# pierre-haessig/stodynprog

Measured on AMD Instinct MI355X. Metric: vi_sweeps_per_sec, higher is better.
Workload: dtype f64

## Files before the change

### stodynprog_amd/codegen.py

```python
import hashlib
import re
import math
import os

import numpy as np

from .trace import TracedModel, DEP_X

CSRC = os.path.join(os.path.dirname(os.path.abspath(__file__)), 'csrc')


DEBUG_INT_MACROS = ('SDP_COL_SHARE_X2', 'SDP_COL_MIN_WAVES', 'SDP_COL_BATCH', 'SDP_COL_WMODE', 'SDP_COL_UNROLL_U', 'SDP_COL_UNROLL_W',
                    'SDP_COL_A_GROUP', 'SDP_COL_A_ORDER', 'SDP_COL_FILTER_UNROLL', 'SDP_COL_B_PRIO',
                    'SDP_COL_FILTER_TOP2', 'SDP_COL_TILE', 'SDP_COL_FILTER_RUNROLL', 'SDP_COL_LEAN', 'SDP_COL_WIDE',
                    'SDP_COL_A_WIDE_LOADS', 'SDP_COLU_WIDE_LOADS', 'SDP_COLU_A_GROUP', 'SDP_COL_LDS_PAD', 'SDP_COL_HOIST',
                    'SDP_COL_TAIL_KEEP', 'SDP_COL_KEEP_BATCH', 'SDP_COL_KEEP_LOADS', 'SDP_COL_TAIL_HOLD', 'SDP_SHORT_GROUP', 'SDP_BNB_CHUNK')
DEBUG_NAMES = frozenset(DEBUG_INT_MACROS + (
    'SDP_STAMP', 'SDP_NO_POW2', 'SDP_EXTRA_DEFINES', 'SDP_COL_FILTER_SCALE', 'SDP_LEAD_FILTER_SCALE',
    'SDP_LEAD_UNROLL', 'SDP_COL_A_LW', 'SDP_COL_FILTER', 'SDP_COL_SHIFT', 'SDP_COL_UTAB', 'SDP_LEAD_FILTER',
    'SDP_COL_THREADS', 'SDP_COL_WCHUNK', 'SDP_STG_CU', 'SDP_COL_WPAIR', 'SDP_COL_WRES', 'SDP_COL_LEAN2', 'SDP_COL_BNB',
    'SDP_LINE_FILTER', 'SDP_LINE_FILTER_SCALE', 'SDP_LINE_TOP2'))


def check_debug(debug):
    if not debug:
        return None
    unknown = sorted(set(debug) - DEBUG_NAMES)
    if unknown:
        raise ValueError('unknown debug define(s): {}'.format(', '.join(unknown)))
    return {k: str(v) for k, v in debug.items() if v is not None and str(v) != ''} or None


def _dbg(debug, name, default=None):
    if not debug:
        return default
    v = debug.get(name)
    return default if v is None or str(v) == '' else str(v)

_BIN_INFIX = {'add': '+', 'sub': '-', 'mul': '*', 'div': '/',
              'lt': '<', 'le': '<=', 'gt': '>', 'ge': '>=', 'eq': '==', 'ne': '!=',
              'and': '&&', 'or': '||', 'xor': '!='}
_FUNC1 = {'abs': 'fabs', 'sqrt': 'sqrt', 'floor': 'floor', 'ceil': 'ceil', 'trunc': 'trunc',
          'rint': 'rint', 'exp': 'exp', 'exp2': 'exp2', 'expm1': 'expm1', 'log': 'log',
          'log2': 'log2', 'log10': 'log10', 'log1p': 'log1p', 'sin': 'sin', 'cos': 'cos',
          'tan': 'tan', 'asin': 'asin', 'acos': 'acos', 'atan': 'atan', 'sinh': 'sinh',
          'cosh': 'cosh', 'tanh': 'tanh', 'cbrt': 'cbrt'}
_FUNC2 = {'pow': 'pow', 'atan2': 'atan2', 'hypot': 'hypot', 'fmod': 'fmod',
          'min': 'sdp_npmin', 'max': 'sdp_npmax', 'fmin': 'sdp_npfmin', 'fmax': 'sdp_npfmax',
          'pymod': 'sdp_nppymod', 'floordiv': 'sdp_npfloordiv'}


def real_literal(value):
    if math.isnan(value):
        return '(sdp_real)NAN'
    if math.isinf(value):
        return '(sdp_real)INFINITY' if value > 0 else '(-(sdp_real)INFINITY)'
    return '(sdp_real)({})'.format(float(value).hex())


def _emit_node(n, name, param_index=None):
    a = [name(x) for x in n.args]
    op = n.op
    if op == 'const':
        if param_index is not None and n.id in param_index:
            return 'sdp_model_prm[{}]'.format(param_index[n.id])
        return real_literal(n.value)
    if op == 'bconst':
        return 'true' if n.value else 'false'
    if op == 'var':
# ... 322 lines not shown
    return lines


def _column_lines(model, dtype, column, col_cfg, window, per_control, filtered, utab, debug, wres=0):
    rs = np.dtype(dtype).itemsize
    wpair = use_wpair(model, dtype, debug) and window is None
    shifted = bool(filtered and column_shift_applies(model, dtype, debug=debug))
    lines = ['#define SDP_COST_HAS_W {}'.format(1 if model.cost_depends_on_w else 0),
             '#define SDP_LEAD_HAS_W {}'.format(1 if model.lead_depends_on_w else 0),
             '#define SDP_TRAIL_HAS_U {}'.format(1 if model.trail_depends_on_u else 0),
             '#define SDP_COL_N0 {}'.format(int(column[0])),
             '#define SDP_COL_W {}'.format(max(int(column[1]), 1)),
             '#define SDP_COL_THREADS {}'.format(col_cfg[0]),
             '#define SDP_COL_WPAIR {}'.format(1 if wpair else 0)]
    if wres:
        lines.append('#define SDP_COL_WRES {}         // resident-chunk form: perturbation points the table holds at a time'.format(int(wres)))
        if rs == 8 and shifted and not _dbg(debug, 'SDP_COL_UNROLL_W'):
            lines.append('#define SDP_COL_UNROLL_W 1')
    if filtered and int(col_cfg[0]) <= 256 and not _dbg(debug, 'SDP_COL_MIN_WAVES'):
        if wres:
            lines.append('#define SDP_COL_MIN_WAVES {}    // as many waves per SIMD as the LDS image admits workgroups per CU, at most 4'.format(
                max(1, min(4, (COLUMN_LDS_MAX // int(col_cfg[1])) * int(col_cfg[0]) // 256))))
        else:
            lines.append('#define SDP_COL_MIN_WAVES 1    // small workgroups of the filtered kernel: no register cap')
    if filtered:
        lines.append('#define SDP_COL_FILTER 1')
        if shifted:
            lines += ['#define SDP_COL_SHIFT 1        // x0\' = a(x, u) +- b_1(x_1.., w) +- ..: first pass on the shifted lattice',
                      '#define SDP_COL_SHIFT_TERMS {}'.format(len(model.lead_split()[1])),
                      '#define SDP_COL_SHIFT_CHAIN {}        // additions of a chain of sums that was regrouped (0: the final-sum form)'.format(
                          model.lead_split_chain()[1] if model.lead_split_chain() is not None else 0),
                      '#define SDP_COL_SHIFT_ROWS {}'.format(int(col_cfg[2]))]
        if _dbg(debug, 'SDP_COL_FILTER_SCALE'):
            lines.append('#define SDP_COL_FILTER_SCALE {}'.format(float(_dbg(debug, 'SDP_COL_FILTER_SCALE'))))
    if per_control is None and not _dbg(debug, 'SDP_COL_A_ORDER'):
        wide = column_wide_loads(column[0], dtype, window, debug)
        order = column_build_order(int(col_cfg[0]), column[1], int(window[2]) if window is not None else column[0],
                                   (16 // rs) if wide else 1)
        if order[0] == 2:
            lw = int(_dbg(debug, 'SDP_COL_A_LW') or order[1])
            lines += ['#define SDP_COL_A_ORDER 2',
                      '#define SDP_COL_A_LW {}'.format(lw)]
            if rs == 4 and int(column[0]) >= 512 and not wres and window is None and not _dbg(debug, 'SDP_COL_A_GROUP'):
                lines.append('#define SDP_COL_A_GROUP 8      // table entries per thread whose vertex loads are issued together')
            if wide and not _dbg(debug, 'SDP_COL_A_WIDE_LOADS'):
                lines.append('#define SDP_COL_A_WIDE_LOADS 1')

                if (wres and rs == 8 and not wpair and window is None and _dbg(debug, 'SDP_COL_TAIL_HOLD') is None
                        and not _dbg(debug, 'SDP_COL_TAIL_KEEP')):
                    tail, groups = int(column[1]) - int(wres), int(col_cfg[0]) // lw
                    if (tail > 0 and tail % groups == 0 and int(column[0]) % (2 * lw) == 0
                            and (tail // groups) * (int(column[0]) // (2 * lw)) * 4 <= 32):
                        lines.append('#define SDP_COL_TAIL_HOLD 1    // the tail of the table is built once and held in registers')
    if window is not None:
        lines.append('#define SDP_COL_ROWS {}'.format(int(window[2])))
    if per_control is not None:
        lines.append('#define SDP_COL_WCHUNK {}'.format(int(per_control[2])))
        if int(column[0]) % (16 // rs) == 0 and not _dbg(debug, 'SDP_COLU_WIDE_LOADS'):
            lines.append('#define SDP_COLU_WIDE_LOADS 1')
    for k in DEBUG_INT_MACROS:
        if _dbg(debug, k):
            lines.append('#define {} {}'.format(k, int(_dbg(debug, k))))
    lines += [separable_functions_source(model), '']
    if utab is not None and filtered:
        lines += ['#define SDP_COL_UTAB {}'.format(len(utab[0])),
                  '#define SDP_COL_UTAB_N {}'.format(int(utab[1])),
                  control_table_source(model, utab[0]), '']
        short = None
        if not model.cost_depends_on_w and window is None and per_control is None \
                and _dbg(debug, 'SDP_COL_LEAN2') != '0' and (not shifted or rs == 8):
            if rs == 8 and wres and _dbg(debug, 'SDP_COL_LEAN') != '0':
                short = short_pass_source(model, utab[0], 'SDP_COL_LEAN2')
                if short and _dbg(debug, 'SDP_COL_BNB') != '0':
                    short += ('\n#define SDP_COL_BNB 1          // the short first pass as a certified branch and bound over '
                              'blocks of controls (sdp_lean2_bnb)')

            elif rs == 4 and not wres and _dbg(debug, 'SDP_COL_WIDE') != '0' and _dbg(debug, 'SDP_COL_LEAN') in (None, '0') \
                    and _dbg(debug, 'SDP_COL_FILTER_TOP2') in (None, '1'):
                short = short_pass_source(model, utab[0], 'SDP_COL_WIDE2')
                if short and _dbg(debug, 'SDP_COL_BNB') != '0':
                    short += ('\n#define SDP_COL_BNB 1          // the short wide first pass as a certified branch and bound over '
                              'blocks of controls (sdp_short_bnb)')
                    if int(column[0]) >= 512 and not _dbg(debug, 'SDP_BNB_CHUNK'):
                        short += '\n#define SDP_BNB_CHUNK 4        // blocks whose bounds are evaluated together (see SDP_COL_A_GROUP above)'
        if short:
            lines += [short, '']
    lines += ['#include "sdp_column_kernel.h"    // also brings in sdp_sweep_kernel.h', '']
    return lines


def line_filter_applies(model, dtype, W, debug=None):
    if _dbg(debug, 'SDP_LINE_FILTER', '1') == '0':
        return False
    return bool(model.n_state == 1 and model.n_perturb == 1 and 1 <= int(W) <= 1024 and np.dtype(dtype).itemsize == 8
                and not model.time_dep and model.lead_depends_on_w and not model.cost_depends_on_w
                and model.lead_split() is not None)


def line_functions_source(model):
    a_node, terms = model.lead_split()
    out = []
    lines = ['SDP_DEV sdp_real sdp_model_lead_a(const sdp_real *x, const sdp_real *u, sdp_real t)',
             '{', '    (void)x; (void)u; (void)t;']
    names = _emit_body(model, model.slice_nodes([a_node]), lines)
    lines += ['    return {};'.format(names[a_node.id]), '}']
    out.append('\n'.join(lines))
# ... 264 lines not shown
    else:
        whole = _column_lds(w, w, n0, n_state, rs, threads, reduced=True, utab_values=utab_values)
        part = _column_lds(half, w, n0, n_state, rs, threads, reduced=True, utab_values=utab_values)
    if COLUMN_LDS_MAX // whole < 3 <= COLUMN_LDS_MAX // part:
        return half if RESIDENT_CHUNKS_DEFAULT else 0
    return 0


RESIDENT_CHUNKS_DEFAULT = True


def column_wide_loads(n0, dtype, window, debug=None):
    if _dbg(debug, 'SDP_COL_A_WIDE_LOADS', '1') == '0':
        return False
    rpl = 16 // np.dtype(dtype).itemsize
    if rpl != 2 and _dbg(debug, 'SDP_COL_A_WIDE_LOADS') != '1':
        return False
    return int(n0) % rpl == 0 and window is None


def column_build_order(threads, w, rows, rows_per_lane=1):
    w = max(int(w), 1)
    best = (0, 0, 0.0)
    for lw in ((32, 64, 16, 8) if rows_per_lane > 1 else (64, 32, 16, 8)):
        if lw * rows_per_lane > rows or threads % lw:
            continue
        groups = threads // lw
        util = w / float(-(-w // groups) * groups)
        if util > best[2] + 1e-9:
            best = (2, lw, util)
    return (best[0], best[1]) if best[2] >= 0.85 else (0, 0)


def bnb_words(n_controls):
    n = max(int(n_controls), 1)
    block = 8
    while (n + block - 1) // block > 64:
        block *= 2
    return 4 * ((n + block - 1) // block + 1)


def utab_reals(n_values, n_controls):
    return int(n_values) * int(n_controls) + bnb_words(n_controls) if n_values else 0


def _column_lds(tw, w, rows, n_state, rs, threads, reduced=False, shift=False, shift_rows=0, utab_values=0,
                partial_minima=False):
    dt = n_state - 1
    part = threads if partial_minima else 1
    members = [(rs, tw * rows, 16),
               (rs, w * dt, rs), (rs, w * dt, rs),
               (rs, 1, rs), (rs, 1, rs),
               (rs, part, rs), (4, part, 4),
               (4, w * dt, 4),
               (4, 4, 4), (4, 1, 4), (8, 2, 8),
               (rs, 2 * (int(utab_values) + 4 if utab_values else 2), 16)]
    if reduced or shift:
        per_row = 4 if rs == 4 else (2 if shift else 1)
        members.append((rs, per_row * int(shift_rows if shift else rows), 16))
    if shift:
        members += [(4, 2 * w, 4), (rs, 2 * w, rs), (rs, 2 * w, rs), (4, 8, 4)]
    off = 0
    for size, count, align in members:
        off = (off + align - 1) // align * align + size * int(count)
    return (off + 15) // 16 * 16


def column_percontrol_config(n0, w, n_state, dtype, debug=None):
    rs = np.dtype(dtype).itemsize
    w = max(int(w), 1)
    threads = min(512, max(64, (int(n0) + 63) // 64 * 64))
    wchunk = max(1, min(w, (32 * 1024) // (int(n0) * rs)))
    if _dbg(debug, 'SDP_COL_WCHUNK'):
        wchunk = max(1, min(w, int(_dbg(debug, 'SDP_COL_WCHUNK'))))
    lds = _column_lds(wchunk, w, n0, n_state, rs, threads)
    if lds > COLUMN_LDS_MAX:
        return None
    return threads, lds, wchunk


def column_window_config(n0, w, n_state, dtype, reach_rows):
    rs = np.dtype(dtype).itemsize
    w = max(int(w), 1)
    for threads, wgs in ((512, 2),):
        budget = COLUMN_LDS_MAX // wgs
        fixed = _column_lds(w, w, 0, n_state, rs, threads, partial_minima=True)
        rows = (budget - fixed) // (w * rs)
        rows = min(rows // 32 * 32, n0)
        seg = (rows - int(reach_rows) - 4) // 64 * 64
        if rows >= 128 and seg >= 64:
            return (threads, _column_lds(w, w, rows, n_state, rs, threads, partial_minima=True), int(rows),
                    int(min(seg, n0)))
    return None


def column_lds_bytes(n0, w, n_state, dtype):
    cfg = column_config(n0, w, n_state, dtype)
    return cfg[1] if cfg else COLUMN_LDS_MAX + 1


HIPCC_FLAGS = ['--genco', '--offload-arch=gfx950', '-O3', '-ffp-contract=off',
               '-fno-fast-math', '-std=c++17', '-I', CSRC]


_HEADERS = ('sdp_kernel_args.h', 'sdp_device.h', 'sdp_sweep_kernel.h', 'sdp_column_kernel.h', 'sdp_colfilter_kernel.h', 'sdp_colres_kernel.h',
            'sdp_colfull_kernel.h', 'sdp_colu_kernel.h',
            'sdp_lead_kernel.h', 'sdp_staged_kernel.h')
# ... 97 lines not shown
```

### stodynprog_amd/csrc/sdp_colres_kernel.h

```cpp
#pragma once

static_assert(SDP_COL_LEAN_ON && !SDP_COL_WIDE_ON, "resident chunks: the lean first pass of 8-byte reals");
static_assert(!SDP_COL_TOP2 || SDP_COL_SHIFT, "resident chunks: two carried survivors only on the shifted lattice");
static_assert(SDP_COL_WRES >= 1 && 2 * SDP_COL_WRES >= SDP_COL_W, "resident chunks: at least half of the points resident");
constexpr int SDP_COLRES_K = SDP_COL_TOP2 ? 2 : 1;

#ifndef SDP_COL_TAIL_KEEP
#define SDP_COL_TAIL_KEEP 0
#endif
#if SDP_COL_TAIL_KEEP && (SDP_COL_SHIFT || !SDP_COL_A_WIDE_LOADS || SDP_COL_A_ORDER != 2 || SDP_COL_WPAIR)
#error "SDP_COL_TAIL_KEEP: the plain resident-chunk kernel with 16-byte build loads"
#endif
#ifndef SDP_COL_TAIL_HOLD
#define SDP_COL_TAIL_HOLD 0
#endif
#if SDP_COL_TAIL_HOLD && (!SDP_COL_A_WIDE_LOADS || SDP_COL_A_ORDER != 2 || SDP_COL_WPAIR || SDP_COL_TAIL_KEEP || \
                          (SDP_COL_W - SDP_COL_WRES) % (SDP_COL_THREADS / SDP_COL_A_LW) != 0 || SDP_COL_ROWS % (2 * SDP_COL_A_LW) != 0)
#error "SDP_COL_TAIL_HOLD: the plain resident-chunk kernel with 16-byte build loads, whole rounds of points and rows"
#endif
#if SDP_COL_TAIL_HOLD
typedef sdp_real sdp_held_rows __attribute__((ext_vector_type(2)));
constexpr int SDP_HOLD_WP = SDP_COL_THREADS / SDP_COL_A_LW;
constexpr int SDP_HOLD_NW = (SDP_COL_W - SDP_COL_WRES) / SDP_HOLD_WP;
constexpr int SDP_HOLD_NJ = SDP_COL_ROWS / (2 * SDP_COL_A_LW);
template <bool BUILD>
SDP_DEV void sdp_colres_tail(const SdpSweepArgs &a, const SdpGrid<sdp_real, SDP_DT> &tg, const SdpColShared &s,
                             sdp_held_rows (&held)[SDP_HOLD_NW][SDP_HOLD_NJ])
{
    constexpr int N0 = SDP_COL_ROWS, C = SDP_COL_WRES, LW = SDP_COL_A_LW, NV = 1 << SDP_DT;
    const sdp_real *__restrict__ V = (const sdp_real *)a.V + s.r0;
    const int tid = sdp_col_tid(), rl = tid % LW, wg = tid / LW;
#pragma unroll
    for (int wi = 0; wi < SDP_HOLD_NW; ++wi) {
        const int tw = wg + wi * SDP_HOLD_WP, w = C + tw;
        if (BUILD) {
            int off[SDP_DT];
            sdp_real lam[SDP_DT], oml[SDP_DT];
#pragma unroll
            for (int k = 0; k < SDP_DT; ++k) {
                off[k] = s.w_off[w * SDP_DT + k];
                lam[k] = s.w_lam[w * SDP_DT + k];
                oml[k] = s.w_oml[w * SDP_DT + k];
            }
            int voff[NV];
#pragma unroll
            for (int q = 0; q < NV; ++q) {
                int o = 0;
#pragma unroll
                for (int k = 0; k < SDP_DT; ++k) o += off[k] + (((q >> (SDP_DT - 1 - k)) & 1) ? tg.M[k] : 0);
                voff[q] = o;
            }
            sdp_held_rows vals2[SDP_HOLD_NJ][NV];
#pragma unroll
            for (int j = 0; j < SDP_HOLD_NJ; ++j) {
                const int r = (j * LW + rl) * 2;
#pragma unroll
                for (int q = 0; q < NV; ++q) vals2[j][q] = *(const sdp_held_rows *)(V + r + voff[q]);
            }
#pragma unroll
            for (int j = 0; j < SDP_HOLD_NJ; ++j) {
                sdp_held_rows e;
#pragma unroll
                for (int c = 0; c < 2; ++c) {
                    sdp_real one[NV];
#pragma unroll
                    for (int q = 0; q < NV; ++q) one[q] = vals2[j][q][c];
                    e[c] = SdpColNest<0, false>::run(one, lam, oml, tg.shift);
                }
                held[wi][j] = e;
            }
        }
#pragma unroll
        for (int j = 0; j < SDP_HOLD_NJ; ++j) *(sdp_held_rows *)(s.T + tw * N0 + (j * LW + rl) * 2) = held[wi][j];
    }
}
#endif

#ifndef SDP_DIAG_SKIP
#define SDP_DIAG_SKIP 0
#endif
#define SDP_COLRES_TAIL_BYTES (SDP_COL_TAIL_KEEP ? (SDP_COL_W - SDP_COL_WRES) * SDP_COL_ROWS * (int)sizeof(sdp_real) : 0)

SDP_DEV void sdp_colres_cell(const SdpLeadAxis &l, const sdp_real *x, const sdp_real *u, sdp_real wv, sdp_real t,
                             int &q0, sdp_real &lam0, sdp_real &oml0)
{
    const sdp_real xn0 = sdp_model_lead(x, u, wv, t);
    const sdp_real sn = sdp_div_span<sdp_real>(xn0 - l.smin, l.span, l.rspan, l.pow2);
    const sdp_real p = sn * l.nm1;
    q0 = max(min(sdp_trunc_i32(p), l.ordm2), 0);
    lam0 = p - (sdp_real)q0;
    oml0 = (sdp_real)1 - lam0;
}

struct SdpColresCand {
    sdp_real u[SDP_COLRES_K][SDP_NU], g[SDP_COLRES_K], acc[SDP_COLRES_K];
    sdp_real lam0[SDP_COLRES_K], oml0[SDP_COLRES_K];
    int q0[SDP_COLRES_K], idx[SDP_COLRES_K];
    int n;
};

template <int K>
SDP_DEV void sdp_colres_partial(const sdp_real *T, const SdpColWeights &k, const SdpLeadAxis &l, const sdp_real *x,
                                sdp_real t, const int w_lo, const int w_hi, const int t_base, SdpColresCand &c)
{
    constexpr int N0 = SDP_COL_ROWS;
    constexpr int B = SDP_COL_BATCH;
    const volatile sdp_lds_real *tab = (const volatile sdp_lds_real *)T;
#pragma unroll SDP_COL_UNROLL_W
    for (int w0 = w_lo; w0 < w_hi; w0 += B) {
        sdp_real lo[B][K], hi[B][K];
#if SDP_LEAD_HAS_W
        sdp_real lam_b[B][K], oml_b[B][K];
#endif
#pragma unroll
        for (int b = 0; b < B; ++b)
            if (w0 + b < w_hi) {
#pragma unroll
                for (int j = 0; j < K; ++j) {
#if SDP_LEAD_HAS_W
                    sdp_colres_cell(l, x, c.u[j], SDP_COL_GW(k, w0 + b), t, c.q0[j], lam_b[b][j], oml_b[b][j]);
#endif
                    lo[b][j] = tab[(w0 + b - t_base) * N0 + c.q0[j]];
                    hi[b][j] = tab[(w0 + b - t_base) * N0 + c.q0[j] + 1];
                }
            }
#pragma unroll
// ... 236 lines not shown
    const SdpBox *box_c = nullptr;
    const sdp_real *w_mine = nullptr;
    sdp_real w_hold = (sdp_real)0;
    if (SDP_COL_HOIST) {
        if (!a.box_per_node) {
            sdp_load_box(a, 0, box_hold);
#pragma unroll
            for (int c = 0; c < SDP_NU; ++c) {
                box_hold.lo[c] = sdp_uniform(box_hold.lo[c]); box_hold.hi[c] = sdp_uniform(box_hold.hi[c]);
                box_hold.step[c] = sdp_uniform(box_hold.step[c]); box_hold.delta[c] = sdp_uniform(box_hold.delta[c]);
                box_hold.n[c] = sdp_uniform(box_hold.n[c]);
            }
            box_hold.total = sdp_uniform(box_hold.total);
            box_c = &box_hold;
        }
        if (lane < Wn && !SDP_COL_TAIL_HOLD) { w_hold = ((const sdp_real *)a.wgrid)[lane]; w_mine = &w_hold; }
    }
#if SDP_COL_SHIFT
    if (threadIdx.x < 2) sdp_col_shift_reset(sdp_lds, threadIdx.x);
    __syncthreads();
#endif
    if (unit < u_end) {
        sdp_real xn[SDP_D];
        sdp_col_coords(a, sdp_col_of_unit(a, unit), xn);
        sdp_col_phase_w(a, tg, s, xn, nullptr, t);
#if SDP_COL_UTAB
        sdp_col_phase_u(a, sdp_lds.utab[0], xn, t, 0, 64, box_c, filt.psum, k_rows, x_cap, (double)filt.psum);
#endif
#if SDP_COL_SHIFT
        sdp_col_phase_shift(a, sdp_lds, lead, xn, t, 0);
#endif
    }
    while (unit < u_end) {
        const int64_t col = sdp_col_of_unit(a, unit);
        const int part = (int)((unsigned)unit % (unsigned)a.col_splits);
        const int i_lo = (int)((unsigned)(N0 * part) / (unsigned)a.col_splits);
        const int i_hi = (int)((unsigned)(N0 * (part + 1)) / (unsigned)a.col_splits);
        sdp_real x[SDP_D];
        sdp_col_coords(a, col, x);
        const int r = sdp_col_tid();
        SDP_RES_MARK(tm0);
        __syncthreads();
#if SDP_STAMP == 2
        { const unsigned long long tmb = __builtin_amdgcn_s_memtime(); tm_top += tmb - tm0; tm0 = tmb; }
#endif
        int nx = 0;
        if (wave == waves - 1 && lane == 0) nx = (int)atomicAdd(claim, 1u);
#if SDP_COL_SHIFT
        if (threadIdx.x == 0) sdp_col_shift_reset(sdp_lds, upar ^ 1);
        SdpColShiftCol shc;
        sdp_col_shift_col(sdp_lds, lead, upar, shc);
        sdp_col_shift_zero(sdp_lds, shc);
#endif
#if SDP_COL_TAIL_HOLD
        sdp_held_rows held[SDP_HOLD_NW][SDP_HOLD_NJ];
        sdp_colres_tail<true>(a, tg, s, held);
#else
        if (!(SDP_DIAG_SKIP & 1)) sdp_col_phase_a<false>(a, tg, s, C, R, kept);
#endif
        __syncthreads();
#if SDP_COL_SHIFT
        sdp_col_shift_reduce(a, sdp_lds, filt, shc, parity, upar, C, R);
#else
        sdp_real acc_t = (sdp_real)0, big = (sdp_real)0;
        if (r < N0 && !(SDP_DIAG_SKIP & 1)) {
#pragma unroll SDP_COL_FILTER_RUNROLL
            for (int w = 0; w < R; ++w) {
                const sdp_real v = sdp_lds.T[w * N0 + r];
                acc_t = acc_t + pw[C + w] * v;
                big = sdp_vmax_abs(big, v);
            }
        }
#endif
        __syncthreads();
        if (!(SDP_DIAG_SKIP & 2)) sdp_col_phase_a<false>(a, tg, s, 0, C);
        if (wave == waves - 1 && lane == 0) sdp_lds.next_unit = nx;
        __syncthreads();
        __builtin_amdgcn_s_setprio(SDP_COL_B_PRIO);
#if SDP_COL_SHIFT
        sdp_col_shift_reduce(a, sdp_lds, filt, shc, parity, upar, 0, C);
#else
        {
            sdp_real dmax = (sdp_real)0;
            if (r < N0) {
                sdp_real acc = (sdp_real)0;
#pragma unroll SDP_COL_FILTER_RUNROLL
                for (int w = 0; w < ((SDP_DIAG_SKIP & 2) ? 0 : C); ++w) {
                    const sdp_real v = sdp_lds.T[w * N0 + r];
                    acc = acc + pw[w] * v;
                    big = sdp_vmax_abs(big, v);
                }
                acc = acc + acc_t;
                dmax = acc == acc ? filt.pcap * big + filt.floor : (sdp_real)INFINITY;
                sdp_lds.ad[r] = acc;
            }
            dmax = sdp_wave_max(dmax);
            if (lane == 0) atomicMax(&sdp_lds.dcol[parity], (unsigned long long)__double_as_longlong((double)dmax));
        }
#endif
        (void)r;
        __syncthreads();
        SDP_RES_MARK(tm1);
#if SDP_STAMP == 2
        tm_build += tm1 - tm0;
#endif
        const sdp_real dcol = sdp_col_filter_dcol(sdp_lds, parity);
        parity ^= 1;
        const int64_t next_unit = u_base + sdp_lds.next_unit;
        SdpLeadAxis lead1 = lead;
#if SDP_COL_SHIFT
        lead1.koff = (sdp_real)shc.kmin;
        lead1.ordm2 = shc.ok ? shc.rows - 2 : 0;
#endif
        const int i = i_lo + (int)threadIdx.x;
        const bool live = i < i_hi;
        const int64_t node = col * N0 + (live ? i : i_hi - 1);
        SdpBox box;
        if (box_c) box = *box_c;
        else sdp_load_box(a, node, box);
        sdp_real best = INFINITY;
        sdp_real diag_cnt = (sdp_real)-1;
        (void)diag_cnt;
        int ibest = INT_MAX;
        SdpColresCand cd;
        cd.n = 0;
#pragma unroll
        for (int j = 0; j < SDP_COLRES_K; ++j) {
            cd.acc[j] = cd.g[j] = cd.lam0[j] = cd.oml0[j] = (sdp_real)0;
            cd.q0[j] = 0;
            cd.idx[j] = INT_MAX;
#pragma unroll
            for (int c = 0; c < SDP_NU; ++c) cd.u[j][c] = (sdp_real)0;
        }
        if (live && (SDP_DIAG_SKIP & 4)) {
            x[0] = axis0[i];
            cd.n = 1; cd.idx[0] = 3; ibest = 3;
            sdp_controls_at(box, 3, cd.u[0]);
            cd.g[0] = sdp_model_cost(x, cd.u[0], (sdp_real)0, t);
            sdp_colres_cell(lead, x, cd.u[0], (sdp_real)0, t, cd.q0[0], cd.lam0[0], cd.oml0[0]);
        } else
        if (live) {
            x[0] = axis0[i];
#if SDP_COL_LEAN2 && SDP_COL_SHIFT
            const sdp_real *utab = sdp_lds.utab[upar];
            const sdp_real *ust = utab + SDP_COL_UTAB * SDP_COL_UTAB_N;
            const sdp_real X = sdp_model_lead_x(x, t), K = sdp_model_cost_x(x, t);
            const int bits = 32 - __clz(max(box.total - 1, 1));
            const int mask = (1 << bits) - 1;
            struct { sdp_real f1, f2, f3; int i1, i2; } bd;
            bd.f1 = bd.f2 = bd.f3 = INFINITY;
            int q_e;
            sdp_real lam_lo, lam_hi, b_max = (sdp_real)0;
            if (axis_mode == 2) {
// ... 9 lines not shown
            const sdp_real l_cap = sdp_vmax_abs(sdp_vmax_abs((sdp_real)1, lam_lo), lam_hi);
            const sdp_real h_cap = (((sdp_real)1 + (sdp_real)2 * (l_cap + shc.lc)) * ((sdp_real)3 + shc.es)) * dcol;
            const sdp_real s_node = fma(filt.pcap, fabs(K) + ust[2], h_cap);
            const bool bad = !filt.ok || !shc.ok || !(s_node < SDP_COL_FILTER_LIMIT) ||
                             !(fabs(lam_lo) + fabs(lam_hi) + shc.lc < (sdp_real)1073741824.0) || bits > 24 || box.total > SDP_COL_UTAB_N;
            const sdp_real radius0 = (filt.cu + (sdp_real)(SDP_COL_FILTER_SCALE) * ldexp(SDP_COL_FILTER_EPS, bits + 1)) * s_node;
#if SDP_COL_BNB
            const sdp_real slack = fma((sdp_real)2, radius0, ((sdp_real)12 * SDP_COL_FILTER_EPS) * s_node);
            const bool bnb = fabs(X) < ust[3] && shc.ok;
            if (__all(bnb)) {
                auto ins = [&](double Fq) {
                    bd.f3 = sdp_vmin(bd.f3, sdp_vmax(bd.f2, Fq));
                    bd.f2 = sdp_vmin(bd.f2, sdp_vmax(bd.f1, Fq));
                    bd.f1 = sdp_vmin(bd.f1, Fq);
                };
                if (axis_mode == 2) sdp_short_bnb<2, false>(sdp_lds.ad, utab, filt, lead1, X, k_rows, 0, box.total, mask, slack, guess, ins, diag_cnt, &b_max);
                else if (axis_mode == 1) sdp_short_bnb<1, false>(sdp_lds.ad, utab, filt, lead1, X, k_rows, 0, box.total, mask, slack, guess, ins, diag_cnt, &b_max);
                else sdp_short_bnb<0, false>(sdp_lds.ad, utab, filt, lead1, X, k_rows, 0, box.total, mask, slack, guess, ins, diag_cnt, &b_max);
            } else
#endif
            {
                if (axis_mode == 2) sdp_lean2s_pass1<2>(sdp_lds.ad, utab, filt, lead1, X, box.total, mask, bd.f1, bd.f2, bd.f3, b_max);
                else if (axis_mode == 1) sdp_lean2s_pass1<1>(sdp_lds.ad, utab, filt, lead1, X, box.total, mask, bd.f1, bd.f2, bd.f3, b_max);
                else sdp_lean2s_pass1<0>(sdp_lds.ad, utab, filt, lead1, X, box.total, mask, bd.f1, bd.f2, bd.f3, b_max);
            }
            const sdp_real radius = fma((sdp_real)(SDP_COL_FILTER_SCALE), b_max, radius0);
            bd.i1 = bd.f1 < (sdp_real)INFINITY ? (__double2loint(bd.f1) & mask) : INT_MAX;
            bd.i2 = bd.f2 < (sdp_real)INFINITY ? (__double2loint(bd.f2) & mask) : INT_MAX;
#elif SDP_COL_LEAN2
            const sdp_real *utab = sdp_lds.utab[upar];
            const sdp_real *ust = utab + SDP_COL_UTAB * SDP_COL_UTAB_N;
            const sdp_real X = sdp_model_lead_x(x, t), K = sdp_model_cost_x(x, t);
            const int bits = 32 - __clz(max(box.total - 1, 1));
            const int mask = (1 << bits) - 1;
            struct { sdp_real f1, f2; int i1, i2; } bd;
            bd.f1 = bd.f2 = INFINITY;
            bd.i2 = INT_MAX;
            int q_e;
            sdp_real lam_lo, lam_hi;
            if (axis_mode == 2) {
                sdp_lean2_cell<2>(lead, SDP_LEAN2_LEAD(X, ust[0]), q_e, lam_lo);
                sdp_lean2_cell<2>(lead, SDP_LEAN2_LEAD(X, ust[1]), q_e, lam_hi);
            } else if (axis_mode == 1) {
                sdp_lean2_cell<1>(lead, SDP_LEAN2_LEAD(X, ust[0]), q_e, lam_lo);
                sdp_lean2_cell<1>(lead, SDP_LEAN2_LEAD(X, ust[1]), q_e, lam_hi);
            } else {
                sdp_lean2_cell<0>(lead, SDP_LEAN2_LEAD(X, ust[0]), q_e, lam_lo);
                sdp_lean2_cell<0>(lead, SDP_LEAN2_LEAD(X, ust[1]), q_e, lam_hi);
            }
            const sdp_real l_cap = sdp_vmax_abs(sdp_vmax_abs((sdp_real)1, lam_lo), lam_hi);
            const sdp_real s_node = fma(filt.pcap, fabs(K) + ust[2], ((sdp_real)1 + (sdp_real)2 * l_cap) * dcol);
            const bool bad = !filt.ok || !(s_node < SDP_COL_FILTER_LIMIT) || !(fabs(lam_lo) + fabs(lam_hi) < (sdp_real)1073741824.0) ||
                             bits > 24 || box.total > SDP_COL_UTAB_N;
            const sdp_real radius = (filt.cu + (sdp_real)(SDP_COL_FILTER_SCALE) * ldexp(SDP_COL_FILTER_EPS, bits + 1)) * s_node;
#if SDP_COL_BNB
            const sdp_real slack = fma((sdp_real)2, radius, ((sdp_real)8 * SDP_COL_FILTER_EPS) * s_node);
            const bool bnb = fabs(X) < ust[3];
            if (__all(bnb)) {
                auto ins = [&](double Fq) {
                    bd.f2 = sdp_vmin(bd.f2, sdp_vmax(bd.f1, Fq));
                    bd.f1 = sdp_vmin(bd.f1, Fq);
                };
                if (axis_mode == 2) sdp_short_bnb<2, false>(sdp_lds.ad, utab, filt, lead, X, k_rows, 0, box.total, mask, slack, guess, ins, diag_cnt);
                else if (axis_mode == 1) sdp_short_bnb<1, false>(sdp_lds.ad, utab, filt, lead, X, k_rows, 0, box.total, mask, slack, guess, ins, diag_cnt);
                else sdp_short_bnb<0, false>(sdp_lds.ad, utab, filt, lead, X, k_rows, 0, box.total, mask, slack, guess, ins, diag_cnt);
            } else
#endif
            {
                if (axis_mode == 2) sdp_lean2_pass1<2>(sdp_lds.ad, utab, filt, lead, X, box.total, mask, bd.f1, bd.f2);
                else if (axis_mode == 1) sdp_lean2_pass1<1>(sdp_lds.ad, utab, filt, lead, X, box.total, mask, bd.f1, bd.f2);
                else sdp_lean2_pass1<0>(sdp_lds.ad, utab, filt, lead, X, box.total, mask, bd.f1, bd.f2);
            }
            bd.i1 = bd.f1 < (sdp_real)INFINITY ? (__double2loint(bd.f1) & mask) : INT_MAX;
#else
            SdpColBounds bd;
            bd.f1 = bd.f2 = bd.f3 = INFINITY;
            bd.s_max = bd.s_sum = bd.p_max = bd.b_max = (sdp_real)0;
            bd.i1 = bd.i2 = INT_MAX;
            const sdp_real *utab = sdp_lds.utab[upar];
            const bool plain = SDP_NU == 1 && box.n[0] > 1 && box.step[0] != (sdp_real)0;
            if (plain) {
                if (axis_mode == 2) sdp_col_filter_pass1<true, 2>(sdp_lds.ad, utab, filt, lead1, box, x, t, 0, box.total, bd);
                else if (axis_mode == 1) sdp_col_filter_pass1<true, 1>(sdp_lds.ad, utab, filt, lead1, box, x, t, 0, box.total, bd);
                else sdp_col_filter_pass1<true, 0>(sdp_lds.ad, utab, filt, lead1, box, x, t, 0, box.total, bd);
            } else {
                if (axis_mode == 2) sdp_col_filter_pass1<false, 2>(sdp_lds.ad, utab, filt, lead1, box, x, t, 0, box.total, bd);
                else if (axis_mode == 1) sdp_col_filter_pass1<false, 1>(sdp_lds.ad, utab, filt, lead1, box, x, t, 0, box.total, bd);
                else sdp_col_filter_pass1<false, 0>(sdp_lds.ad, utab, filt, lead1, box, x, t, 0, box.total, bd);
            }
#if SDP_COL_SHIFT
            const sdp_real h_cap = (((sdp_real)1 + (sdp_real)2 * (bd.p_max + shc.lc)) * ((sdp_real)3 + shc.es)) * dcol;
            const sdp_real s_node = fma(filt.ratio, bd.s_sum + h_cap, h_cap);
            const bool bad = !filt.ok || !shc.ok || !(s_node < SDP_COL_FILTER_LIMIT) || !(bd.p_max + shc.lc < (sdp_real)1073741824.0);
            const sdp_real radius = fma(filt.cu, s_node, (sdp_real)(SDP_COL_FILTER_SCALE) * bd.b_max);
#else
            const sdp_real h_cap = ((sdp_real)1 + (sdp_real)2 * bd.p_max) * dcol;
            const sdp_real s_node = fma(filt.ratio, bd.s_sum + h_cap, h_cap);
            const bool bad = !filt.ok || !(s_node < SDP_COL_FILTER_LIMIT) || !(bd.p_max < (sdp_real)1073741824.0);
            const sdp_real radius = filt.cu * s_node;
#endif
#endif
            const sdp_real m_hi = bd.f1 + radius;
            const bool single = !bad && bd.i1 != INT_MAX && bd.f2 - radius > m_hi;
#if SDP_COL_LEAN2 && !SDP_COL_SHIFT
            const bool pair = false;
#else
            const bool pair = SDP_COL_TOP2 && !bad && !single && bd.i2 != INT_MAX && bd.f3 - radius > m_hi;
// ... 3 lines not shown
                cd.idx[0] = single ? bd.i1 : min(bd.i1, bd.i2);
                if (SDP_COLRES_K > 1) cd.idx[SDP_COLRES_K - 1] = single ? bd.i1 : max(bd.i1, bd.i2);
                else ibest = bd.i1;
#pragma unroll
                for (int j = 0; j < SDP_COLRES_K; ++j) {
                    sdp_controls_at(box, cd.idx[j], cd.u[j]);
                    cd.g[j] = sdp_model_cost(x, cd.u[j], (sdp_real)0, t);
#if !SDP_LEAD_HAS_W
                    sdp_colres_cell(lead, x, cd.u[j], (sdp_real)0, t, cd.q0[j], cd.lam0[j], cd.oml0[j]);
#endif
                }
            } else {
                for (int ci = 0; ci < box.total; ++ci) {
                    sdp_real u[SDP_NU];
                    sdp_controls_at(box, ci, u);
                    bool cand = bad;
                    if (!cand) {
#if SDP_COL_LEAN2 && SDP_COL_SHIFT
                        sdp_real b_unused = (sdp_real)0;
                        const sdp_real F = lead.pow2 ? sdp_lean2s_value<1>(sdp_lds.ad, utab, filt, lead1, X, ci, b_unused)
                                                     : sdp_lean2s_value<0>(sdp_lds.ad, utab, filt, lead1, X, ci, b_unused);
#elif SDP_COL_LEAN2
                        const sdp_real F = lead.pow2 ? sdp_lean2_value<1>(sdp_lds.ad, utab, filt, lead, X, ci)
                                                     : sdp_lean2_value<0>(sdp_lds.ad, utab, filt, lead, X, ci);
#else
                        sdp_real F, pm = (sdp_real)0, gm = (sdp_real)0, bm = (sdp_real)0;
                        if (lead.pow2) sdp_col_lean_eval<1>(sdp_lds.ad, filt, lead1, x, u, t, F, pm, gm, bm);
                        else sdp_col_lean_eval<0>(sdp_lds.ad, filt, lead1, x, u, t, F, pm, gm, bm);
#endif
                        cand = !(F - radius > m_hi);
                    }
                    if (cand) {
                        const sdp_real jc = sdp_col_cost_global<false>(a, tg, s, wts, lead, x, u, t);
                        if (ibest == INT_MAX || sdp_better_seq(jc, best)) { best = jc; ibest = ci; }
                    }
                }
            }
        }
#if SDP_STAMP == 2
        tm_p1 += __builtin_amdgcn_s_memtime() - tm1;
#endif
        const bool two = SDP_COLRES_K > 1 && __any(cd.n == 2);
        if (SDP_DIAG_SKIP & 8) {}
        else if (SDP_COLRES_K > 1 && two) sdp_colres_partial<SDP_COLRES_K>(sdp_lds.T, wts, lead, x, t, 0, C, 0, cd);
        else if (cd.n) sdp_colres_partial<1>(sdp_lds.T, wts, lead, x, t, 0, C, 0, cd);
#if SDP_COL_TAIL_KEEP
        if (cd.n) sdp_colres_partial_kept(kept, wts, C, Wn, cd);
#ifdef SDP_DIAG_KEEP_BARRIER
        __syncthreads();
#endif
#else
        __syncthreads();
        __builtin_amdgcn_s_setprio(0);
#if SDP_COL_TAIL_HOLD
        sdp_colres_tail<false>(a, tg, s, held);
#else
        if (!(SDP_DIAG_SKIP & 16)) sdp_col_phase_a<false>(a, tg, s, C, R);
#endif
        __syncthreads();
        __builtin_amdgcn_s_setprio(SDP_COL_B_PRIO);
        if (SDP_DIAG_SKIP & 32) {}
        else if (SDP_COLRES_K > 1 && two) sdp_colres_partial<SDP_COLRES_K>(sdp_lds.T, wts, lead, x, t, C, Wn, C, cd);
        else if (cd.n) sdp_colres_partial<1>(sdp_lds.T, wts, lead, x, t, C, Wn, C, cd);
#endif
        if (live) {
#pragma unroll
            for (int j = 0; j < SDP_COLRES_K; ++j) {
                if (SDP_COLRES_K == 1) { if (cd.n) best = cd.acc[0]; }
                else if (j < cd.n && (ibest == INT_MAX || sdp_better_seq(cd.acc[j], best))) { best = cd.acc[j]; ibest = cd.idx[j]; }
            }
#ifdef SDP_DIAG_BNB_COUNT
            best = diag_cnt;
#endif
            if (!(SDP_DIAG_SKIP & 128)) sdp_col_store(a, node, box, best, ibest);
            if (ibest != INT_MAX) guess = ibest;
        }
        {
            const int nxu = __builtin_amdgcn_readfirstlane(sdp_lds.next_unit);
            if (u_base + nxu < u_end && !(SDP_DIAG_SKIP & 64)) {
                sdp_real xn[SDP_D];
                sdp_col_coords(a, sdp_col_of_unit(a, u_base + nxu), xn);
                sdp_col_phase_w(a, tg, s, xn, nullptr, t, (waves - 1) * 64, 64, w_mine);
#if SDP_COL_UTAB
                sdp_col_phase_u(a, sdp_lds.utab[upar ^ 1], xn, t, max(waves - 2, 0) * 64, 64, box_c, filt.psum, k_rows, x_cap, (double)filt.psum,
                                SDP_LEAN2_A_FIXED_ON && tables_made >= 2);
                ++tables_made;
#endif
#if SDP_COL_SHIFT
                sdp_col_phase_shift(a, sdp_lds, lead, xn, t, upar ^ 1, max(waves - 3, 0) * 64, 64);
#endif
            }
        }
        __builtin_amdgcn_s_setprio(0);
        upar ^= 1;
        unit = next_unit;
    }
    if (threadIdx.x == 0) {
        __threadfence();
        if (atomicAdd(a.claim + 256, 1u) == gridDim.x - 1) {
            for (int k = 0; k < 8; ++k) atomicExch(a.claim + 32 * k, 0u);
            atomicExch(a.claim + 256, 0u);
        }
    }
#if SDP_STAMP == 2
    if (a.stamps && (threadIdx.x & 63) == 0) {
        tm_all = __builtin_amdgcn_s_memtime() - tm_start;
        unsigned long long *o = a.stamps + ((size_t)blockIdx.x * (blockDim.x >> 6) + (threadIdx.x >> 6)) * 4;
// ... 66 lines not shown
```

### stodynprog_amd/csrc/sdp_column_kernel.h

```cpp
#pragma once
#include "sdp_sweep_kernel.h"
#include <type_traits>

#if SDP_D >= 2

#ifndef SDP_COL_THREADS
#define SDP_COL_THREADS 512
#endif
#ifndef SDP_COL_UNROLL_W
#define SDP_COL_UNROLL_W 4
#endif
#ifndef SDP_COL_A_GROUP
#define SDP_COL_A_GROUP 4
#endif
#ifndef SDP_COL_A_ORDER
#define SDP_COL_A_ORDER 0
#endif
#ifndef SDP_COL_A_LW
#define SDP_COL_A_LW 16
#endif
#ifndef SDP_COLU_WIDE_LOADS
#define SDP_COLU_WIDE_LOADS 0
#endif
#ifndef SDP_COLU_A_GROUP
// ... 109 lines not shown
#define SDP_COL_HOIST 1
#endif
#if SDP_COL_FILTER && (!SDP_HAS_W || (SDP_LEAD_HAS_W && !SDP_COL_SHIFT) || SDP_TRAIL_HAS_U || SDP_COL_ROWS < SDP_COL_N0)
#error "SDP_COL_FILTER needs a perturbation that reaches x0' through a final sum at most, and the plain full-column table"
#endif
#if SDP_COL_SHIFT && (!SDP_COL_FILTER || !SDP_LEAD_HAS_W || SDP_COL_WPAIR)
#error "SDP_COL_SHIFT is a form of the certified filter for a perturbation that reaches x0'"
#endif
#if SDP_COL_FILTER && SDP_COST_HAS_W && SDP_COL_UTAB
#error "the control table holds sub-expressions without the perturbation: not with a cost that depends on it"
#endif
#if SDP_TRAIL_HAS_U && (SDP_COL_WPAIR || SDP_COL_ROWS < SDP_COL_N0)
#error "control-dependent trailing dynamics: plain full table, exact arithmetic only"
#endif
#if SDP_COL_ROWS < SDP_COL_N0 && SDP_COL_WPAIR
#error "the row window is built for the plain table layout with exact arithmetic"
#endif
constexpr bool SDP_COL_WINDOW = SDP_COL_ROWS < SDP_COL_N0;
constexpr int SDP_DT = SDP_D - 1;
constexpr int SDP_COL_TW = SDP_COL_WPAIR ? (SDP_COL_W + 1) / 2 * 2 : SDP_COL_W;

#ifndef SDP_COL_WMODE
#define SDP_COL_WMODE 1
#endif
struct SdpColShared {
    sdp_real *T;
    int *w_off;
    sdp_real *w_lam;
    sdp_real *w_oml;
    sdp_real *part_J;
    int *part_i;
    int r0;
};

#ifndef SDP_COL_WCHUNK
#define SDP_COL_WCHUNK SDP_COL_W
#endif
constexpr int SDP_COL_LDS_WCOPY = SDP_COL_WMODE == 2 ? SDP_COL_W : 1;
constexpr int SDP_COL_LDS_PART = (SDP_COL_FILTER || SDP_TRAIL_HAS_U) ? 1 : SDP_COL_THREADS;
constexpr int SDP_BNB_BLOCK = sdp_bnb_block(SDP_COL_UTAB_N);
constexpr int SDP_BNB_BLOCKS = (SDP_COL_UTAB_N + SDP_BNB_BLOCK - 1) / SDP_BNB_BLOCK;
constexpr int SDP_BNB_WORDS = SDP_COL_UTAB ? 4 * (SDP_BNB_BLOCKS + 1) : 0;
#define SDP_AD_A(ad, r) (SDP_COL_WIDE2 ? ((double *)(ad))[(r)] : *(double *)((ad) + 4 * (r)))
#define SDP_AD_A_CONST(ad, r) (SDP_COL_WIDE2 ? ((const double *)(ad))[(r)] : *(const double *)((ad) + 4 * (r)))
constexpr int SDP_COL_LDS_AD = sizeof(SDP_REAL) == 4 ? 4 : ((SDP_COL_LEAN != 0 && !SDP_COL_SHIFT) ? 1 : 2);
struct __attribute__((aligned(16))) SdpColLds {
    sdp_real T[(SDP_TRAIL_HAS_U ? SDP_COL_WCHUNK : (SDP_COL_WRES < SDP_COL_W ? SDP_COL_WRES : SDP_COL_TW)) * SDP_COL_ROWS];
    sdp_real w_lam[SDP_COL_W * SDP_DT];
    sdp_real w_oml[SDP_COL_W * SDP_DT];
    sdp_real pw[SDP_COL_LDS_WCOPY];
    sdp_real gw[SDP_COL_LDS_WCOPY];
    sdp_real part_J[SDP_COL_LDS_PART];
    int part_i[SDP_COL_LDS_PART];
    int w_off[SDP_COL_W * SDP_DT];
    int win[2][2];
    int next_unit;
    unsigned long long dcol[2];
    sdp_real utab[2][SDP_COL_UTAB ? SDP_COL_UTAB * SDP_COL_UTAB_N + 4 + SDP_BNB_WORDS : 2] __attribute__((aligned(16)));
#if SDP_COL_LDS_PAD
    char pad_[SDP_COL_LDS_PAD];
#endif
#if SDP_COL_FILTER
    sdp_real ad[SDP_COL_LDS_AD * (SDP_COL_SHIFT ? SDP_COL_SHIFT_ROWS : SDP_COL_ROWS)] __attribute__((aligned(16)));
#endif
#if SDP_COL_SHIFT
    int sh_q[2][SDP_COL_W];
    sdp_real sh_f[2][SDP_COL_W];
    sdp_real sh_c[2][SDP_COL_W];
    int sh_k[2][4];
#endif
};
static_assert(sizeof(SdpColLds) <= 160 * 1024, "column table exceeds the 160 KiB LDS of a CU");

struct SdpColDiag {
    unsigned long long m1 = 0, m2 = 0, tp1 = 0, tp2 = 0, n_slow = 0, n_exact = 0, n_all = 0;
};
#if SDP_STAMP == 2
#define SDP_COL_MARK(v) v = __builtin_amdgcn_s_memtime()
#else
#define SDP_COL_MARK(v)
#endif

SDP_DEV void sdp_col_carve(SdpColLds &m, SdpColShared &s)
{
    s.T = m.T;
    s.w_lam = m.w_lam;
    s.w_oml = m.w_oml;
    s.w_off = m.w_off;
    s.part_J = m.part_J;
    s.part_i = m.part_i;
    s.r0 = 0;
}

SDP_DEV double sdp_uniform_real(double v) { return __hiloint2double(__builtin_amdgcn_readfirstlane(__double2hiint(v)), __builtin_amdgcn_readfirstlane(__double2loint(v))); }
SDP_DEV float sdp_uniform_real(float v) { return __int_as_float(__builtin_amdgcn_readfirstlane(__float_as_int(v))); }
SDP_DEV void sdp_col_trailing_grid(const SdpSweepArgs &a, SdpGrid<sdp_real, SDP_DT> &g)
{
    const sdp_real *axes = (const sdp_real *)a.axes;
    int m = SDP_COL_N0;
    g.pow2 = 0;
#pragma unroll
    for (int k = SDP_DT - 1; k >= 0; --k) {
        const int ax = k + 1;
        g.smin[k] = axes[a.axis_off[ax]];
        g.span[k] = axes[a.axis_off[ax] + a.orders[ax] - 1] - g.smin[k];
        g.rspan[k] = (sdp_real)1 / g.span[k];
        if (sdp_is_pow2(g.span[k])) g.pow2 |= 1 << k;
// ... 801 lines not shown
```

Before: 895.1.

## Fuse head and tail table builds into one phase with in-wave reduction

Adds a one-build path for the resident-chunk column kernel. The head chunk and the held tail are built in a single pass, and each half-wave handles alternating points for a row pair. The weighted sum is reduced across halves with a lane shuffle, so the separate phase-A reduction and one barrier round are no longer needed. It is enabled automatically for two trailing axes, unshifted lattices and N0 equal to the thread count. The cost is extra register pressure and a narrower set of configurations where it applies.

```diff
diff --git a/stodynprog_amd/codegen.py b/stodynprog_amd/codegen.py
--- a/stodynprog_amd/codegen.py
+++ b/stodynprog_amd/codegen.py
@@ -14,7 +14,8 @@
                     'SDP_COL_A_GROUP', 'SDP_COL_A_ORDER', 'SDP_COL_FILTER_UNROLL', 'SDP_COL_B_PRIO',
                     'SDP_COL_FILTER_TOP2', 'SDP_COL_TILE', 'SDP_COL_FILTER_RUNROLL', 'SDP_COL_LEAN', 'SDP_COL_WIDE',
                     'SDP_COL_A_WIDE_LOADS', 'SDP_COLU_WIDE_LOADS', 'SDP_COLU_A_GROUP', 'SDP_COL_LDS_PAD', 'SDP_COL_HOIST',
-                    'SDP_COL_TAIL_KEEP', 'SDP_COL_KEEP_BATCH', 'SDP_COL_KEEP_LOADS', 'SDP_COL_TAIL_HOLD', 'SDP_SHORT_GROUP', 'SDP_BNB_CHUNK')
+                    'SDP_COL_TAIL_KEEP', 'SDP_COL_KEEP_BATCH', 'SDP_COL_KEEP_LOADS', 'SDP_COL_TAIL_HOLD', 'SDP_SHORT_GROUP', 'SDP_BNB_CHUNK',
+                    'SDP_COL_ONE_BUILD', 'SDP_ONE_GROUP')
 DEBUG_NAMES = frozenset(DEBUG_INT_MACROS + (
     'SDP_STAMP', 'SDP_NO_POW2', 'SDP_EXTRA_DEFINES', 'SDP_COL_FILTER_SCALE', 'SDP_LEAD_FILTER_SCALE',
     'SDP_LEAD_UNROLL', 'SDP_COL_A_LW', 'SDP_COL_FILTER', 'SDP_COL_SHIFT', 'SDP_COL_UTAB', 'SDP_LEAD_FILTER',
@@ -443,6 +444,10 @@
                     if (tail > 0 and tail % groups == 0 and int(column[0]) % (2 * lw) == 0
                             and (tail // groups) * (int(column[0]) // (2 * lw)) * 4 <= 32):
                         lines.append('#define SDP_COL_TAIL_HOLD 1    // the tail of the table is built once and held in registers')
+                        if (not shifted and int(column[0]) == int(col_cfg[0]) and int(col_cfg[0]) % 64 == 0
+                                and int(wres) % 2 == 0 and tail % 2 == 0 and tail <= 16 and model.n_state == 3
+                                and _dbg(debug, 'SDP_COL_ONE_BUILD') is None):
+                            lines.append('#define SDP_COL_ONE_BUILD 1    // head and tail in one build phase, A reduced inside each wave')
     if window is not None:
         lines.append('#define SDP_COL_ROWS {}'.format(int(window[2])))
     if per_control is not None:
@@ -813,7 +818,7 @@
                (rs, w * dt, rs), (rs, w * dt, rs),
                (rs, 1, rs), (rs, 1, rs),
                (rs, part, rs), (4, part, 4),
-               (4, w * dt, 4),
+               (4, w * dt, 8),
                (4, 4, 4), (4, 1, 4), (8, 2, 8),
                (rs, 2 * (int(utab_values) + 4 if utab_values else 2), 16)]
     if reduced or shift:
diff --git a/stodynprog_amd/csrc/sdp_colres_kernel.h b/stodynprog_amd/csrc/sdp_colres_kernel.h
--- a/stodynprog_amd/csrc/sdp_colres_kernel.h
+++ b/stodynprog_amd/csrc/sdp_colres_kernel.h
@@ -72,6 +72,70 @@
         }
 #pragma unroll
         for (int j = 0; j < SDP_HOLD_NJ; ++j) *(sdp_held_rows *)(s.T + tw * N0 + (j * LW + rl) * 2) = held[wi][j];
+    }
+}
+#endif
+
+#ifndef SDP_COL_ONE_BUILD
+#define SDP_COL_ONE_BUILD 0
+#endif
+#if SDP_COL_ONE_BUILD && (!SDP_COL_TAIL_HOLD || SDP_COL_SHIFT || SDP_COL_N0 != SDP_COL_THREADS || \
+                          SDP_COL_WRES % 2 != 0 || (SDP_COL_W - SDP_COL_WRES) % 2 != 0 || SDP_COL_W - SDP_COL_WRES > 16 || \
+                          SDP_COL_THREADS % 64 != 0)
+#error "SDP_COL_ONE_BUILD: the held tail without the shifted lattice, a lane per row pair (N0 = threads), two trailing axes, even chunks"
+#endif
+#ifndef SDP_ONE_GROUP
+#define SDP_ONE_GROUP 2
+#endif
+#if SDP_COL_ONE_BUILD
+static_assert(SDP_DT == 2, "SDP_COL_ONE_BUILD: two trailing axes (a cell's record: two offsets, two weights)");
+constexpr int SDP_ONE_HN = SDP_COL_WRES / 2;
+constexpr int SDP_ONE_TN = (SDP_COL_W - SDP_COL_WRES) / 2;
+template <int N>
+SDP_DEV void sdp_colres_one_run(const sdp_real *__restrict__ V, const SdpGrid<sdp_real, SDP_DT> &tg, const SdpColShared &s,
+                                const sdp_cst_real *pw, const int w0, const int h, const int r, sdp_held_rows *held,
+                                sdp_held_rows &acc, sdp_real &big)
+{
+    constexpr int N0 = SDP_COL_ROWS, NV = 1 << SDP_DT, G = SDP_ONE_GROUP;
+#pragma unroll
+    for (int g0 = 0; g0 < N; g0 += G) {
+        sdp_held_rows vals[G][NV];
+        int wg[G];
+#pragma unroll
+        for (int g = 0; g < G; ++g)
+            if (g0 + g < N) {
+                const int w = w0 + 2 * (g0 + g) + h;
+                wg[g] = w;
+                const int2 off = *(const int2 *)(s.w_off + w * SDP_DT);
+                const int base = r + off.x + off.y;
+#pragma unroll
+                for (int q = 0; q < NV; ++q)
+                    vals[g][q] = *(const sdp_held_rows *)(V + base + ((q & 2) ? tg.M[0] : 0) + ((q & 1) ? tg.M[1] : 0));
+            }
+#pragma unroll
+        for (int g = 0; g < G; ++g)
+            if (g0 + g < N) {
+                const sdp_held_rows lam2 = *(const sdp_held_rows *)(s.w_lam + wg[g] * SDP_DT);
+                const sdp_held_rows oml2 = *(const sdp_held_rows *)(s.w_oml + wg[g] * SDP_DT);
+                const sdp_real lam[SDP_DT] = {lam2.x, lam2.y}, oml[SDP_DT] = {oml2.x, oml2.y};
+                sdp_held_rows e;
+#pragma unroll
+                for (int c = 0; c < 2; ++c) {
+                    sdp_real one[NV];
+#pragma unroll
+                    for (int q = 0; q < NV; ++q) one[q] = vals[g][q][c];
+                    e[c] = SdpColNest<0, false>::run(one, lam, oml, tg.shift);
+                }
+                if (held) held[g0 + g] = e;
+                else *(sdp_held_rows *)(s.T + wg[g] * N0 + r) = e;
+                const volatile sdp_cst_real *pv = pw;
+                const sdp_real p0 = pv[w0 + 2 * (g0 + g)], p1 = pv[w0 + 2 * (g0 + g) + 1];
+                const sdp_real p = h ? p1 : p0;
+                acc.x = acc.x + p * e.x;
+                acc.y = acc.y + p * e.y;
+                big = sdp_vmax_abs(sdp_vmax_abs(big, e.x), e.y);
+            }
+        __builtin_amdgcn_sched_barrier(0);
     }
 }
 #endif
@@ -414,6 +478,29 @@
         sdp_col_shift_col(sdp_lds, lead, upar, shc);
         sdp_col_shift_zero(sdp_lds, shc);
 #endif
+#if SDP_COL_ONE_BUILD
+        sdp_held_rows held[SDP_ONE_TN];
+        {
+            const int tid = sdp_col_tid(), h = (tid >> 5) & 1, rp = (tid & ~63) + 2 * (tid & 31);
+            const sdp_real *__restrict__ Vb = (const sdp_real *)a.V + s.r0;
+            sdp_held_rows acc2 = (sdp_real)0;
+            sdp_real big = (sdp_real)0;
+            if (!(SDP_DIAG_SKIP & 2)) sdp_colres_one_run<SDP_ONE_HN>(Vb, tg, s, pw, 0, h, rp, nullptr, acc2, big);
+            if (!(SDP_DIAG_SKIP & 1)) sdp_colres_one_run<SDP_ONE_TN>(Vb, tg, s, pw, C, h, rp, held, acc2, big);
+            else {
+#pragma unroll
+                for (int j = 0; j < SDP_ONE_TN; ++j) held[j] = (sdp_real)0;
+            }
+            const sdp_real acc = (h ? acc2.y : acc2.x) + __shfl_xor(h ? acc2.x : acc2.y, 32);
+            sdp_real dmax = acc == acc ? filt.pcap * big + filt.floor : (sdp_real)INFINITY;
+            sdp_lds.ad[rp + h] = acc;
+            dmax = sdp_wave_max(dmax);
+            if (lane == 0) atomicMax(&sdp_lds.dcol[parity], (unsigned long long)__double_as_longlong((double)dmax));
+        }
+        if (wave == waves - 1 && lane == 0) sdp_lds.next_unit = nx;
+        __builtin_amdgcn_s_setprio(SDP_COL_B_PRIO);
+        (void)r;
+#else
 #if SDP_COL_TAIL_HOLD
         sdp_held_rows held[SDP_HOLD_NW][SDP_HOLD_NJ];
         sdp_colres_tail<true>(a, tg, s, held);
@@ -461,6 +548,7 @@
         }
 #endif
         (void)r;
+#endif
         __syncthreads();
         SDP_RES_MARK(tm1);
 #if SDP_STAMP == 2
@@ -576,7 +664,8 @@
             const sdp_real s_node = fma(filt.pcap, fabs(K) + ust[2], ((sdp_real)1 + (sdp_real)2 * l_cap) * dcol);
             const bool bad = !filt.ok || !(s_node < SDP_COL_FILTER_LIMIT) || !(fabs(lam_lo) + fabs(lam_hi) < (sdp_real)1073741824.0) ||
                              bits > 24 || box.total > SDP_COL_UTAB_N;
-            const sdp_real radius = (filt.cu + (sdp_real)(SDP_COL_FILTER_SCALE) * ldexp(SDP_COL_FILTER_EPS, bits + 1)) * s_node;
+            const sdp_real radius = (filt.cu + (sdp_real)(SDP_COL_FILTER_SCALE) *
+                                     ldexp(SDP_COL_FILTER_EPS, (SDP_COL_ONE_BUILD ? sdp_col_opaque(bits) : bits) + 1)) * s_node;
 #if SDP_COL_BNB
             const sdp_real slack = fma((sdp_real)2, radius, ((sdp_real)8 * SDP_COL_FILTER_EPS) * s_node);
             const bool bnb = fabs(X) < ust[3];
@@ -686,7 +775,13 @@
 #else
         __syncthreads();
         __builtin_amdgcn_s_setprio(0);
-#if SDP_COL_TAIL_HOLD
+#if SDP_COL_ONE_BUILD
+        {
+            const int tid = sdp_col_tid(), h = (tid >> 5) & 1, rp = (tid & ~63) + 2 * (tid & 31);
+#pragma unroll
+            for (int j = 0; j < SDP_ONE_TN; ++j) *(sdp_held_rows *)(sdp_lds.T + (2 * j + h) * N0 + rp) = held[j];
+        }
+#elif SDP_COL_TAIL_HOLD
         sdp_colres_tail<false>(a, tg, s, held);
 #else
         if (!(SDP_DIAG_SKIP & 16)) sdp_col_phase_a<false>(a, tg, s, C, R);
diff --git a/stodynprog_amd/csrc/sdp_column_kernel.h b/stodynprog_amd/csrc/sdp_column_kernel.h
--- a/stodynprog_amd/csrc/sdp_column_kernel.h
+++ b/stodynprog_amd/csrc/sdp_column_kernel.h
@@ -185,7 +185,7 @@
     sdp_real gw[SDP_COL_LDS_WCOPY];
     sdp_real part_J[SDP_COL_LDS_PART];
     int part_i[SDP_COL_LDS_PART];
-    int w_off[SDP_COL_W * SDP_DT];
+    int w_off[SDP_COL_W * SDP_DT] __attribute__((aligned(8)));
     int win[2][2];
     int next_unit;
     unsigned long long dcol[2];
```

After: 906.1 (median of 6 runs). 1.01x the previous value.
